# nadongjun/mirbft

Measured on AMD Instinct MI355X. Metric: SHA-256 digests/s (request + batch digests), Actions.Hash stream, higher is better.
Workload: dtype u32

## Files before the change

mirbft_amd/csrc/mirsha_ctx.h:

```cpp
#pragma once
#include <hip/hip_runtime.h>

#include <algorithm>
#include <atomic>
#include <chrono>
#include <condition_variable>
#include <cstdarg>
#include <cstdio>
#include <cstdlib>
#include <cstring>
#include <functional>
#include <mutex>
#include <string>
#include <thread>
#include <vector>

#include "../../include/mirsha.h"
#include "mirsha_host.h"
#include "mirsha_device.h"
#include "mirsha_order.h"
#include "mirsha_sha512.h"
#include "mirsha_sha512_pair.h"
#include "mirsha_sha512_plan.h"

// ... 210 lines not shown
    PinnedBuf stage;
    DevBuf dev, d_out;
    RingOwner ring;
};

struct mirsha_pipeline {
    int device = 0;
    int mode = MIRSHA_PIPELINE_FUSED;
    int hasher = MIRSHA_HASHER_SHA256;
    uint32_t n_req = 0, n_lists = 0, n_entries = 0;
    std::vector<uint32_t> tadj_first, tadj, cbase, expected;
    uint32_t n_tiles = 0, n_groups = 0, n_counters = 0, grid = 0;
    uint32_t pace = 1, list_blocks = 0, tile_waves = 0;
    uint32_t list_tiles = 0;
    uint32_t q_first[mirsha::kFusedMaxQueues + 1] = {};
    uint32_t q_end[mirsha::kFusedMaxQueues] = {};
    uint32_t q_waves[mirsha::kFusedMaxQueues] = {};
    uint32_t tile_blocks = 0;
    uint64_t epoch = 0;
    DevBuf d_tadj_first, d_tadj, d_cbase, d_expected, d_counters, d_ctl, d_trace;
    unsigned long long* h_err = nullptr;
    unsigned long long* d_err = nullptr;
    unsigned long long watchdog = mirsha::kFusedWatchdogTicks;
    uint32_t n_split = 0, split_first = 0, seg_per_tile = 0, seg_nominal_nb = 0;
    std::vector<uint32_t> seg_nb;
    DevBuf d_seg_nb, d_seg_state, d_seg_flags;
    uint64_t seg_runs = 0;
    int fallback = 0;
    uint32_t test_placement = 0;
    DevBuf d_probe;
    bool trace = false;
    std::vector<uint32_t> cidx, cfirst;
    uint32_t uniform = 0;
    std::vector<uint32_t> order;
    DevBuf d_cidx, d_cfirst, d_order;
};

namespace mirsha_api {

int fail(mirsha_ctx* c, int code, const char* fmt, ...);

#define HIP_TRY(c, expr)                                                                    \
    do {                                                                                    \
        hipError_t _e = (expr);                                                             \
        if (_e != hipSuccess)                                                               \
            return fail((c), _e == hipErrorOutOfMemory ? MIRSHA_ENOMEM : MIRSHA_EHIP,       \
                        "%s: %s (%s:%d)", #expr, hipGetErrorString(_e), __FILE__, __LINE__); \
    } while (0)

hipEvent_t take_event(KernelTimer& t);

template <class F>
int timed_launch(mirsha_ctx* c, int which, F&& launch) {
    hipEvent_t e0 = nullptr, e1 = nullptr;
    const bool timed = c->timing && ((c->time_mask >> which) & 1u);
    if (timed) {
        e0 = take_event(c->timers[which]);
        e1 = take_event(c->timers[which]);
        if (e0 && e1) mirsha::next_launch_events() = {e0, e1};
    }
    hipError_t e = launch();
    const bool bound = e0 && e1 && !mirsha::next_launch_events().start;
    mirsha::next_launch_events() = {};
    if (timed && (!bound || e != hipSuccess)) {
        if (e0) c->timers[which].pool.push_back(e0);
        if (e1) c->timers[which].pool.push_back(e1);
    }
    if (e != hipSuccess) return fail(c, MIRSHA_EHIP, "kernel launch: %s", hipGetErrorString(e));
    if (bound) c->timers[which].pending.emplace_back(e0, e1);
    return MIRSHA_OK;
}

inline hipError_t hasher_launch_msgs(const mirsha_ctx* c, const uint8_t* arena, uint64_t arena_len,
                                     const uint64_t* off, const uint32_t* len, const uint32_t* order, uint32_t n,
                                     uint8_t* out, hipStream_t s) {
    if (c->hasher == MIRSHA_HASHER_SHA512_256)
        return mirsha::launch_sha512_msgs(arena, arena_len, off, len, order, n, out, c->variant, s,
                                          &c->sha512_pair_launches);
    return mirsha::launch_msgs(arena, arena_len, off, len, order, n, out, c->variant, s);
}
inline hipError_t hasher_launch_lists(const mirsha_ctx* c, const uint8_t* digests, uint32_t n_digests,
                                      const uint32_t* idx, uint32_t n_entries, const uint32_t* first, uint32_t n_lists,
                                      uint32_t* scratch, uint8_t* out, hipStream_t s) {
    if (c->hasher == MIRSHA_HASHER_SHA512_256)
        return mirsha::launch_sha512_lists(digests, n_digests, idx, n_entries, first, n_lists, scratch, out, s,
                                           &c->sha512_pair_launches);
    return mirsha::launch_lists(digests, n_digests, idx, n_entries, first, n_lists, scratch, out, s);
}

inline const char* hasher_name(int hasher) { return hasher == MIRSHA_HASHER_SHA512_256 ? "sha512_256" : "sha256"; }

inline int sha256_only(mirsha_ctx* c, const char* call) {
    if (!c || c->hasher == MIRSHA_HASHER_SHA256) return MIRSHA_OK;
    return fail(c, MIRSHA_EINVAL, "%s: hasher %s is not built for this call", call, hasher_name(c->hasher));
}

inline int chains_hasher_match(mirsha_ctx* c, const mirsha_chains* ch, const char* call) {
    if (!c || !ch || c->hasher == ch->hasher) return MIRSHA_OK;
    return fail(c, MIRSHA_EINVAL, "%s: the chains hash with %s, the context with %s", call, hasher_name(ch->hasher),
                hasher_name(c->hasher));
}

inline int plan_hasher_match(mirsha_ctx* c, const mirsha_pipeline* p, const char* call) {
    if (!c || !p || c->hasher == p->hasher) return MIRSHA_OK;
    return fail(c, MIRSHA_EINVAL, "%s: the plan hashes with %s, the context with %s", call, hasher_name(p->hasher),
                hasher_name(c->hasher));
}

inline int streams_hasher_match(mirsha_ctx* c, const mirsha_streams* st, const char* call) {
    if (!c || !st || c->hasher == st->hasher) return MIRSHA_OK;
    return fail(c, MIRSHA_EINVAL, "%s: the streams hash with %s, the context with %s", call, hasher_name(st->hasher),
                hasher_name(c->hasher));
// ... 230 lines not shown
```

mirbft_amd/csrc/mirsha_kernels.h:

```cpp
#pragma once
#include <hip/hip_runtime.h>
#include <stdint.h>

namespace mirsha {

constexpr uint32_t kWavesPerBlock = 4;
constexpr uint32_t kBlockThreads = 64 * kWavesPerBlock;
constexpr uint32_t kNullIndex = 0xFFFFFFFFu;

enum : int {
    kVariantLds = 0,
    kVariantDirect = 1,
    kVariantLowOcc = 4,
    kVariantLdsOnly = 5,
    kVariantPair = 6,
    kVariantCu = 10,
};
const char* ab_getenv(const char* name);
inline bool variant_valid(int v) {
    return v == kVariantLds || v == kVariantDirect || v == kVariantLowOcc || v == kVariantLdsOnly || v == kVariantPair ||
           v == kVariantCu;
}
constexpr uint32_t kCuMaxWavesPerSimd = 4;
uint32_t cu_count();
constexpr uint32_t kLowOccTiles = 1024;
constexpr uint32_t kPairMaxGroups = 512;
uint32_t pair_max_groups();

constexpr uint64_t kMaxBufferArena = 0xFFFFFF00ull;
constexpr uint32_t kMaxBufferMsgs = 1u << 27;
hipError_t launch_offsets_scan(void* tmp, size_t& tmp_bytes, const uint32_t* len, uint64_t* off, uint32_t n,
                               hipStream_t s);
struct LaunchEvents {
    hipEvent_t start = nullptr, stop = nullptr;
};
LaunchEvents& next_launch_events();

hipError_t launch_msgs(const uint8_t* arena, uint64_t arena_len, const uint64_t* off,
                       const uint32_t* len, const uint32_t* order, uint32_t n, uint8_t* out,
                       int variant, hipStream_t s);
constexpr uint32_t kMaxListDigests = (1u << 27) - 1u;
constexpr uint32_t kMaxListEntries = (1u << 30) - 1u;
hipError_t launch_lists(const uint8_t* digests, uint32_t n_digests, const uint32_t* idx, uint32_t n_entries,
                        const uint32_t* first, uint32_t n_lists, uint32_t* scratch, uint8_t* out, hipStream_t s);
struct PadBlockKW {
    uint32_t kw[64];
    uint32_t use;
};
PadBlockKW pad_block_kw(uint64_t L);
hipError_t launch_chain(const uint8_t* digests, uint32_t n_digests, const uint32_t* cidx, uint32_t n_entries,
                        const uint32_t* cfirst, uint32_t n_lists, uint8_t* out, hipStream_t s, uint32_t uniform = 0);
hipError_t launch_chain_pair(const uint8_t* digests, uint32_t n_digests, const uint32_t* cidx, uint32_t n_entries,
                             const uint32_t* cfirst, uint32_t n_lists, uint8_t* out, hipStream_t s);
struct OverlapArgs {
    const uint8_t* arena;
    uint64_t arena_len;
    const uint64_t* off;
    const uint32_t* len;
    const uint32_t* order;
    uint32_t n_req;
    uint8_t* req_out;
    const uint8_t* prev_digests;
    uint32_t n_req_prev;
    const uint32_t* cidx;
    uint32_t n_entries;
    const uint32_t* cfirst;
    uint32_t n_lists;
    uint8_t* list_out;
    uint32_t list_waves;
    uint32_t chain_prio;
};
hipError_t launch_msgs_overlap(const OverlapArgs& a, hipStream_t s);
constexpr uint32_t kFusedChunkBlocks = 2;
// ... 63 lines not shown
```

mirbft_amd/csrc/mirsha_kernels.hip:

```cpp
#include <algorithm>
#include <atomic>
#include <cstdlib>
#include <cstdio>
#include <type_traits>

#include "mirsha_device.h"

namespace mirsha {

struct RawChunk {
    uint32_t v[5];
    uint32_t sel;
};

__device__ __forceinline__ void issue_chunk(__amdgpu_buffer_rsrc_t rsrc, uint32_t records, uint32_t o,
                                            uint32_t blk, uint32_t q, bool active, RawChunk& c) {
    const uint32_t addr = o + 64u * blk + 16u * q;
    const uint32_t a = active ? (addr & ~3u) : 0xFFFFFFE0u;
    c.sel = be_sel(addr & 3u);
    if (a + 20u <= records || !active) {
        const auto v = __builtin_amdgcn_raw_buffer_load_b128(rsrc, a, 0, 0);
        c.v[0] = v[0]; c.v[1] = v[1]; c.v[2] = v[2]; c.v[3] = v[3];
        c.v[4] = __builtin_amdgcn_raw_buffer_load_b32(rsrc, a + 16u, 0, 0);
    } else {
        asm volatile(
            "s_nop 4\n\t"
            "buffer_load_dword %0, %5, %6, 0 offen\n\t"
            "buffer_load_dword %1, %5, %6, 0 offen offset:4\n\t"
            "buffer_load_dword %2, %5, %6, 0 offen offset:8\n\t"
            "buffer_load_dword %3, %5, %6, 0 offen offset:12\n\t"
            "buffer_load_dword %4, %5, %6, 0 offen offset:16\n\t"
            "s_waitcnt vmcnt(0)"
            : "=&v"(c.v[0]), "=&v"(c.v[1]), "=&v"(c.v[2]), "=&v"(c.v[3]), "=&v"(c.v[4])
            : "v"(a), "s"(rsrc)
// ... 11 lines not shown
    for (int k = 0; k < 5; k++) c.v[k] = 0u;
    if (active) {
        const uint32_t* p = reinterpret_cast<const uint32_t*>(arena + a);
        if (a + 20u <= records) {
            const u32x4a4 v = *reinterpret_cast<const u32x4a4*>(p);
            c.v[0] = v[0]; c.v[1] = v[1]; c.v[2] = v[2]; c.v[3] = v[3];
            c.v[4] = p[4];
        } else {
#pragma unroll
            for (int k = 0; k < 5; k++)
                if (a + 4u * k + 4u <= records) c.v[k] = p[k];
        }
    }
}

__device__ __forceinline__ void pad_words(uint32_t p, uint32_t L, bool last_block, uint32_t q, uint32_t out[4]) {
    if (p + 16u > L) {
#pragma unroll
        for (int k = 0; k < 4; k++) {
            const int32_t t = (int32_t)(L - (p + 4u * k));
            const uint32_t sh = (uint32_t)t << 3;
            const uint32_t keep = ~(0xFFFFFFFFu >> sh);
            const uint32_t mark = 0x80000000u >> sh;
            const uint32_t part = (out[k] & keep) | mark;
            out[k] = t >= 4 ? out[k] : (t < 0 ? 0u : part);
        }
        if (last_block && q == 3u) {
            out[2] = L >> 29;
            out[3] = L << 3;
        }
    }
}

template <int kWords = 16>
__device__ __forceinline__ void pad_block_uniform(uint32_t w[16], uint32_t soff, uint32_t L, bool last) {
#pragma unroll
    for (int k = 0; k < kWords; k++) {
        const int32_t t = (int32_t)(L - (soff + 4u * k));
        const uint32_t sh = (uint32_t)t << 3;
        uint32_t keep = t >= 4 ? 0xFFFFFFFFu : (t <= 0 ? 0u : ~(0xFFFFFFFFu >> sh));
        uint32_t mark = (t >= 0 && t < 4) ? 0x80000000u >> sh : 0u;
        if (k >= 14 && last) {
            keep = 0u;
            mark = k == 14 ? L >> 29 : L << 3;
        }
        keep = __builtin_amdgcn_readfirstlane(keep);
        mark = __builtin_amdgcn_readfirstlane(mark);
        w[k] = (w[k] & keep) | mark;
    }
}

__device__ __forceinline__ void finish_chunk(const RawChunk& c, uint32_t p, uint32_t L, bool last_block,
                                             uint32_t q, uint32_t out[4]) {
#pragma unroll
    for (int k = 0; k < 4; k++) out[k] = be_word(c.v[k + 1], c.v[k], c.sel);
    pad_words(p, L, last_block, q, out);
}

__device__ __forceinline__ uint32_t lds_slot(uint32_t m, uint32_t q) {
    return m * 4u + (q ^ ((m >> 2) & 3u));
}

__device__ __forceinline__ void store_digest_buf(__amdgpu_buffer_rsrc_t ors, uint32_t msg, const uint32_t st[8]) {
    __builtin_amdgcn_raw_buffer_store_b128(
        (uint32_t __attribute__((ext_vector_type(4)))){__builtin_bswap32(st[0]), __builtin_bswap32(st[1]),
                                                        __builtin_bswap32(st[2]), __builtin_bswap32(st[3])},
        ors, 32u * msg, 0, 0);
    __builtin_amdgcn_raw_buffer_store_b128(
        (uint32_t __attribute__((ext_vector_type(4)))){__builtin_bswap32(st[4]), __builtin_bswap32(st[5]),
                                                        __builtin_bswap32(st[6]), __builtin_bswap32(st[7])},
// ... 90 lines not shown
    asm volatile("s_mov_b32 %0, %1" : "=s"(wnb) : "s"(wave_nb));
    return wnb - blk == 1u;
}

template <bool kFused, bool kBuf>
__device__ __forceinline__ void tile_store(uint8_t* out, uint32_t n, uint32_t msg, const uint32_t st[8]) {
    if constexpr (kFused || kBuf) {
        const __amdgpu_buffer_rsrc_t ors =
            __builtin_amdgcn_make_buffer_rsrc((void*)out, (short)0, (int)(32u * n), 0x00020000);
        if constexpr (kFused)
            store_digest_sc1(ors, msg, st);
        else
            store_digest_buf(ors, msg, st);
    } else {
        store_digest(out, msg, st);
    }
}

template <bool kFused>
__device__ __forceinline__ void block_prio(uint32_t fprio, uint32_t blk) {
    if constexpr (kFused) {
        if (fprio == kPrioBalance)
            balance_prio(blk);
        else if (fprio == kPrioProgress)
            progress_prio(blk);
        else
            fixed_prio(fprio);
    } else {
        progress_prio(blk);
    }
}

constexpr uint32_t kTilePaused = 0, kTileDone = 1;
template <bool kLds, bool kWide, bool kFused = false, bool kDma = false>
__device__ __forceinline__ uint32_t hash_tile(const uint8_t* __restrict__ arena, uint64_t arena_len,
                                          const uint64_t* __restrict__ off, const uint32_t* __restrict__ len,
                                          const uint32_t* __restrict__ order, uint32_t n, uint8_t* __restrict__ out,
                                          uint4* my, uint32_t t, uint32_t lane, uint32_t fprio = 0,
                                          uint32_t b0 = 0u, uint32_t b1 = 0xFFFFFFFFu, uint32_t* st_io = nullptr,
                                          uint32_t lone_sel = 0u, uint4* my2 = nullptr,
                                          unsigned long long* lone_tr = nullptr) {
    __builtin_amdgcn_s_setprio(3);
    const uint32_t slot = t * 64u + lane;
    const bool valid = slot < n;
    const uint32_t slot_c = valid ? slot : n - 1u;
    const uint32_t msg = order ? order[slot_c] : slot_c;
    const uint32_t L_ = len[msg];
    const uint64_t o_ = off[msg];
    const uint32_t L = valid ? L_ : 0u;
    const uint64_t o = valid ? o_ : 0u;
    const uint32_t nb = valid ? blocks_for_len(L) : 0u;
    const uint32_t max_l = wave_max(valid ? L : 0u);
    const uint32_t wave_nb = blocks_for_len(max_l);

    const uint64_t records = (arena_len + 3u) & ~3ull;
    const __amdgpu_buffer_rsrc_t rsrc =
        __builtin_amdgcn_make_buffer_rsrc((void*)arena, (short)0, (int)(uint32_t)records, 0x00020000);
    auto issue = [&](uint64_t mo, uint32_t blk, uint32_t q, bool active, RawChunk& rc) {
        if constexpr (kWide)
            issue_chunk_wide(arena, records, mo, blk, q, active, rc);
        else
            issue_chunk(rsrc, (uint32_t)records, (uint32_t)mo, blk, q, active, rc);
    };

    uint32_t st[8];
#pragma unroll
    for (int i = 0; i < 8; i++) st[i] = (st_io && b0) ? st_io[i] : kH0[i];
    const bool finished = b1 >= wave_nb;

    if constexpr (kLds && !kWide) {
        const uint32_t q = lane & 3u;
        const uint64_t reach = valid ? o + 64ull * wave_nb + 20u : 0ull;
        const bool far = __builtin_amdgcn_ballot_w64(reach > records) == 0;
        const bool aligned = __builtin_amdgcn_ballot_w64(valid && (o & 3u) != 0u) == 0;
        const uint32_t min_l = wave_min(valid ? L : 0xFFFFFFFFu);
        const bool uni = max_l == min_l;
        const int32_t u_last = (int32_t)(min_l - 64u * (wave_nb - 1u));
        const bool tail_ok = uni && u_last <= 16;
        const TailWords tw = tail_words(u_last, min_l);
        uint32_t vo[4], sel[4];
#pragma unroll
        for (int j = 0; j < 4; j++) {
            const uint32_t a = (uint32_t)__shfl((int)(uint32_t)o, 16 * j + (int)(lane >> 2), 64) + 16u * q;
            vo[j] = a & ~3u;
            sel[j] = be_sel(a & 3u);
        }
        auto stage = [&](uint32_t blk, uint32_t w[16], uint32_t ln, bool trim) {
            const uint32_t soff = 64u * blk;
            const uint32_t qq = ln & 3u;
            const bool skip = trim && soff + 16u * qq >= min_l;
            RawChunk rc[4];
            if (far && !trim) {
#pragma unroll
                for (int j = 0; j < 4; j++) {
                    const auto v = __builtin_amdgcn_raw_buffer_load_b128(rsrc, vo[j], soff, 0);
                    rc[j].v[0] = v[0]; rc[j].v[1] = v[1]; rc[j].v[2] = v[2]; rc[j].v[3] = v[3];
                    rc[j].v[4] = 0u;
                }
                if (!aligned) {
#pragma unroll
                    for (int j = 0; j < 4; j++)
                        rc[j].v[4] = __builtin_amdgcn_raw_buffer_load_b32(rsrc, vo[j], soff + 16u, 0);
                }
            } else if (far) {
#pragma unroll
                for (int j = 0; j < 4; j++) {
                    const uint32_t a = skip ? 0xFFFFFFE0u : vo[j] + soff;
                    const auto v = __builtin_amdgcn_raw_buffer_load_b128(rsrc, a, 0, 0);
                    rc[j].v[0] = v[0]; rc[j].v[1] = v[1]; rc[j].v[2] = v[2]; rc[j].v[3] = v[3];
                    rc[j].v[4] = aligned ? 0u : __builtin_amdgcn_raw_buffer_load_b32(rsrc, a + 16u, 0, 0);
                }
// ... 134 lines not shown
            uint32_t w[16];
#pragma unroll
            for (int k = 0; k < 4; k++) {
                const uint4 x = my[lds_slot(lane, (uint32_t)k)];
                w[4 * k + 0] = x.x; w[4 * k + 1] = x.y; w[4 * k + 2] = x.z; w[4 * k + 3] = x.w;
            }
            wave_lds_handoff();
            progress_prio(blk);
            if (blk < nb) compress_asm(st, w);
        }
    } else {
        for (uint32_t blk = 0; blk < wave_nb; blk++) {
            const bool active = blk < nb;
            RawChunk rc[4];
#pragma unroll
            for (int q = 0; q < 4; q++) issue(o, blk, (uint32_t)q, active, rc[q]);
            uint32_t w[16];
#pragma unroll
            for (int q = 0; q < 4; q++)
                finish_chunk(rc[q], 64u * blk + 16u * q, L, blk + 1u == nb, (uint32_t)q, &w[4 * q]);
            progress_prio(blk);
            if (active) compress_asm(st, w);
        }
    }
    if (!finished) {
#pragma unroll
        for (int i = 0; i < 8; i++) st_io[i] = st[i];
        return kTilePaused;
    }
    if (valid) tile_store<kFused, kLds && !kWide>(out, n, msg, st);
    return kTileDone;
}

constexpr uint32_t kMsgWaves = 1;
constexpr uint32_t kMsgOcc = 8, kTileSlots = 256;
template <bool kLds, bool kWide = false>
__global__ __launch_bounds__(64 * kMsgWaves, kWide ? 6 : kMsgOcc) void sha256_msgs_kernel(
    const uint8_t* __restrict__ arena, uint64_t arena_len, const uint64_t* __restrict__ off,
    const uint32_t* __restrict__ len, const uint32_t* __restrict__ order, uint32_t n,
    uint8_t* __restrict__ out) {
    __shared__ uint4 tile[kMsgWaves][kTileSlots];
    const uint32_t lane = threadIdx.x & 63u;
    const uint32_t wv = threadIdx.x >> 6;
    const uint32_t t = blockIdx.x * kMsgWaves + wv;
    if (t * 64u >= n) return;
    hash_tile<kLds, kWide>(arena, arena_len, off, len, order, n, out, tile[wv], t, lane);
}

constexpr uint32_t kCuLds = 96u * 1024u;
__global__ __launch_bounds__(1024, 1) void sha256_msgs_cu_kernel(const uint8_t* __restrict__ arena,
                                                                 uint64_t arena_len,
                                                                 const uint64_t* __restrict__ off,
                                                                 const uint32_t* __restrict__ len,
                                                                 const uint32_t* __restrict__ order, uint32_t n,
                                                                 uint8_t* __restrict__ out) {
    extern __shared__ uint4 cu_lds[];
    const uint32_t lane = threadIdx.x & 63u;
    const uint32_t wv = threadIdx.x >> 6;
    const uint32_t t = blockIdx.x * (blockDim.x >> 6) + wv;
    if (t * 64u >= n) return;
    hash_tile<true, false, false, true>(arena, arena_len, off, len, order, n, out, cu_lds + 256u * wv, t, lane);
}

__device__ __forceinline__ void overlap_chain(const uint8_t* __restrict__ digests, uint32_t n_digests,
                                              const uint32_t* __restrict__ cidx, uint32_t n_entries,
                                              const uint32_t* __restrict__ cfirst, uint32_t n_lists,
                                              uint8_t* __restrict__ list_out, uint32_t g, uint32_t lane,
                                              uint32_t prio_mode) {
    __builtin_amdgcn_s_setprio(3);
    const uint32_t k = g * 64u + lane;
    const bool valid = k < n_lists;
    const uint32_t kc = valid ? k : n_lists - 1u;
    const uint32_t e0_ = cfirst[kc], e1_ = cfirst[kc + 1];
    const uint32_t e0 = valid ? e0_ : 0u;
    const uint32_t c = valid ? e1_ - e0_ : 0u;
    const uint32_t L = 32u * c;
    const uint32_t nb = valid ? blocks_for_len(L) : 0u;
    const uint32_t wave_nb = blocks_for_len(32u * wave_max(c));
    const __amdgpu_buffer_rsrc_t drs = buffer_rsrc(digests, 32u * n_digests);
// ... 886 lines not shown
        const char* m = ab_getenv("MIRSHA_PAIR_MAX_GROUPS");
        return m ? (uint32_t)strtoul(m, nullptr, 10) : kPairMaxGroups;
    }();
    return v;
}

uint32_t cu_count() {
    static std::atomic<uint32_t> cached[64] = {};
    int dev = 0;
    if (hipGetDevice(&dev) != hipSuccess || dev < 0 || dev >= 64) return 256u;
    uint32_t v = cached[dev].load(std::memory_order_relaxed);
    if (!v) {
        int a = 0;
        if (hipDeviceGetAttribute(&a, hipDeviceAttributeMultiprocessorCount, dev) != hipSuccess || a <= 0) a = 256;
        v = (uint32_t)a;
        cached[dev].store(v, std::memory_order_relaxed);
    }
    return v;
}

enum DynLdsKernel { kDynLdsCu, kDynLdsFused, kDynLdsProbe, kDynLdsKernels };
hipError_t dyn_lds_attr(const void* fn, DynLdsKernel form, uint32_t bytes) {
    static std::atomic<uint8_t> done[64][kDynLdsKernels] = {};
    int dev = 0;
    if (hipError_t e = hipGetDevice(&dev)) return e;
    if (dev >= 0 && dev < 64 && done[dev][form].load(std::memory_order_acquire)) return hipSuccess;
    if (hipError_t e = hipFuncSetAttribute(fn, hipFuncAttributeMaxDynamicSharedMemorySize, (int)bytes)) return e;
    if (dev >= 0 && dev < 64) done[dev][form].store(1, std::memory_order_release);
    return hipSuccess;
}

hipError_t launch_msgs(const uint8_t* arena, uint64_t arena_len, const uint64_t* off,
                       const uint32_t* len, const uint32_t* order, uint32_t n, uint8_t* out,
                       int variant, hipStream_t s) {
    if (n == 0) return hipSuccess;
    const uint32_t tiles = (n + 63u) / 64u;
    const uint32_t grid = (tiles + kWavesPerBlock - 1u) / kWavesPerBlock;
    const uint32_t mgrid = (tiles + kMsgWaves - 1u) / kMsgWaves;
    if (arena_len > kMaxBufferArena || n >= kMaxBufferMsgs) {
        launch_k(sha256_msgs_kernel<true, true>, mgrid, 64 * kMsgWaves, 0, s, arena, arena_len, off, len, order, n, out);
        return hipGetLastError();
    }
    if (variant == kVariantPair || (variant == kVariantLds && tiles <= pair_max_groups())) {
        launch_k(sha256_msgs_pair_kernel, tiles, kPairThreads, 0, s, arena, arena_len, off, len, order, n, out);
        return hipGetLastError();
    }
    if (variant == kVariantLowOcc || (variant == kVariantLds && tiles <= kLowOccTiles)) {
        launch_k(sha256_msgs_lowocc_kernel, grid, kBlockThreads, 0, s, arena, arena_len, off, len, order, n, out);
        return hipGetLastError();
    }
    if (variant == kVariantCu || (variant == kVariantLds && tiles <= kCuMaxWavesPerSimd * 4u * cu_count())) {
        const uint32_t k = (tiles + 4u * cu_count() - 1u) / (4u * cu_count());
        const uint32_t wg_waves = 4u * std::min(k, kCuMaxWavesPerSimd);
        const uint32_t cgrid = (tiles + wg_waves - 1u) / wg_waves;
        if (hipError_t e = dyn_lds_attr((const void*)sha256_msgs_cu_kernel, kDynLdsCu, kCuLds)) return e;
        launch_k(sha256_msgs_cu_kernel, cgrid, 64u * wg_waves, kCuLds, s, arena, arena_len, off, len, order, n, out);
        return hipGetLastError();
    }
    if (variant == kVariantDirect)
        launch_k(sha256_msgs_kernel<false>, mgrid, 64 * kMsgWaves, 0, s, arena, arena_len, off, len, order, n, out);
    else
        launch_k(sha256_msgs_kernel<true>, mgrid, 64 * kMsgWaves, 0, s, arena, arena_len, off, len, order, n, out);
    return hipGetLastError();
}

hipError_t launch_msgs_overlap(const OverlapArgs& a, hipStream_t s) {
    const uint32_t tiles = (a.n_req + 63u) / 64u;
    if (a.list_waves + tiles == 0) return hipSuccess;
    if (a.arena_len > kMaxBufferArena || a.n_req >= kMaxBufferMsgs || (a.list_waves && a.n_lists == 0))
        return hipErrorInvalidValue;
    launch_k(sha256_msgs_overlap_kernel, a.list_waves + tiles, 64, 0, s, a);
    return hipGetLastError();
}

hipError_t launch_lists(const uint8_t* digests, uint32_t n_digests, const uint32_t* idx, uint32_t n_entries,
                        const uint32_t* first, uint32_t n_lists, uint32_t* scratch, uint8_t* out, hipStream_t s) {
    if (n_lists == 0) return hipSuccess;
    const uint32_t grid = (n_lists + kBlockThreads - 1u) / kBlockThreads;
    launch_k(sha256_lists_kernel, grid, kBlockThreads, 0, s, digests, n_digests, idx, n_entries, first, n_lists, scratch,
                                                      out);
    return hipGetLastError();
}

PadBlockKW pad_block_kw(uint64_t L) {
    auto rotr = [](uint32_t x, int n) { return (x >> n) | (x << (32 - n)); };
    uint32_t w[64] = {0x80000000u};
    w[14] = (uint32_t)(L >> 29);
    w[15] = (uint32_t)(L << 3);
    for (int j = 16; j < 64; j++) {
        const uint32_t s0 = rotr(w[j - 15], 7) ^ rotr(w[j - 15], 18) ^ (w[j - 15] >> 3);
        const uint32_t s1 = rotr(w[j - 2], 17) ^ rotr(w[j - 2], 19) ^ (w[j - 2] >> 10);
        w[j] = w[j - 16] + s0 + w[j - 7] + s1;
    }
    PadBlockKW p{};
    for (int j = 0; j < 64; j++) p.kw[j] = kK[j] + w[j];
// ... 103 lines not shown
```

mirbft_amd/csrc/mirsha_plan.hip:

```cpp
#include "mirsha_ctx.h"

namespace mirsha_api {

uint32_t uniform_lists(const std::vector<uint32_t>& cidx, const std::vector<uint32_t>& cfirst) {
    const size_t n_lists = cfirst.size() - 1, n = cidx.size();
    if (n_lists == 0 || n == 0 || cfirst[1] == 0) return 0;
    const uint64_t B = cfirst[1];
    if ((n_lists - 1) * B >= n || n_lists * B < n) return 0;
    for (size_t k = 0; k < n_lists; k++)
        if (cfirst[k] != k * B) return 0;
    for (size_t e = 0; e < n; e++)
        if (cidx[e] != e) return 0;
    if (const char* e = mirsha::ab_getenv("MIRSHA_CHAIN_UNIFORM"))
        if (e[0] == '0') return 0;
    return (uint32_t)B;
}

int pipeline_build(mirsha_ctx* c, mirsha_pipeline* p, uint32_t n_req, const uint32_t* idx, const uint32_t* first,
                   uint32_t n_lists, const uint32_t* len) {
    p->n_req = n_req;
    p->n_lists = n_lists;
    p->cfirst.assign(n_lists + 1, 0);
    p->cidx.clear();
    p->cidx.reserve(first[n_lists]);
    std::vector<uint8_t> listed(n_req, 0);
    for (uint32_t k = 0; k < n_lists; k++) {
        for (uint32_t e = first[k]; e < first[k + 1]; e++) {
            if (idx[e] == MIRSHA_NULL_INDEX) continue;
            p->cidx.push_back(idx[e]);
            listed[idx[e]] = 1;
        }
        p->cfirst[k + 1] = (uint32_t)p->cidx.size();
    }
    p->n_entries = (uint32_t)p->cidx.size();
    p->uniform = uniform_lists(p->cidx, p->cfirst);
    p->order.resize(n_req);
    for (uint32_t r = 0; r < n_req; r++) p->order[r] = r;
    std::stable_sort(p->order.begin(), p->order.end(), [&](uint32_t x, uint32_t y) {
        if (listed[x] != listed[y]) return listed[x] > listed[y];
        return len ? host_blocks(len[x]) > host_blocks(len[y]) : false;
    });
    HIP_TRY(c, p->d_cidx.ensure(sizeof(uint32_t) * std::max<uint32_t>(p->n_entries, 1)));
    HIP_TRY(c, p->d_cfirst.ensure(sizeof(uint32_t) * (n_lists + 1)));
    HIP_TRY(c, p->d_order.ensure(sizeof(uint32_t) * std::max<uint32_t>(n_req, 1)));
    if (p->n_entries)
        HIP_TRY(c, hipMemcpyAsync(p->d_cidx.p, p->cidx.data(), sizeof(uint32_t) * p->n_entries, hipMemcpyHostToDevice, c->stream));
    HIP_TRY(c, hipMemcpyAsync(p->d_cfirst.p, p->cfirst.data(), sizeof(uint32_t) * (n_lists + 1), hipMemcpyHostToDevice, c->stream));
    if (n_req)
        HIP_TRY(c, hipMemcpyAsync(p->d_order.p, p->order.data(), sizeof(uint32_t) * n_req, hipMemcpyHostToDevice, c->stream));
    HIP_TRY(c, hipStreamSynchronize(c->stream));
    return MIRSHA_OK;
}

struct PlanKernels {
    hipError_t (*requests)(const mirsha_ctx* c, const mirsha_pipeline* p, const uint8_t* d_arena, uint64_t arena_len,
                           const uint64_t* d_off, const uint32_t* d_len, uint8_t* d_req_out);
    hipError_t (*lists)(const mirsha_ctx* c, const mirsha_pipeline* p, const uint8_t* d_digests, uint8_t* d_list_out);
    hipError_t (*overlap)(const mirsha_ctx* c, const mirsha_pipeline* p, bool tiles, bool chains,
                          const uint8_t* d_arena, uint64_t arena_len, const uint64_t* d_off, const uint32_t* d_len,
                          uint8_t* d_req_out, const uint8_t* d_prev_req, uint8_t* d_prev_batch_out);
};

const PlanKernels kPlanSha256 = {
    [](const mirsha_ctx* c, const mirsha_pipeline* p, const uint8_t* d_arena, uint64_t arena_len, const uint64_t* d_off,
       const uint32_t* d_len, uint8_t* d_req_out) {
        return mirsha::launch_msgs(d_arena, arena_len, d_off, d_len, p->d_order.as<uint32_t>(), p->n_req, d_req_out,
                                   c->variant, c->stream);
    },
    [](const mirsha_ctx* c, const mirsha_pipeline* p, const uint8_t* d_digests, uint8_t* d_list_out) {
        if ((p->n_lists + 63u) / 64u <= mirsha::pair_max_groups())
            return mirsha::launch_chain_pair(d_digests, p->n_req, p->d_cidx.as<uint32_t>(), p->n_entries,
                                             p->d_cfirst.as<uint32_t>(), p->n_lists, d_list_out, c->stream);
        return mirsha::launch_chain(d_digests, p->n_req, p->d_cidx.as<uint32_t>(), p->n_entries,
                                    p->d_cfirst.as<uint32_t>(), p->n_lists, d_list_out, c->stream, p->uniform);
    },
    [](const mirsha_ctx* c, const mirsha_pipeline* p, bool tiles, bool chains, const uint8_t* d_arena,
       uint64_t arena_len, const uint64_t* d_off, const uint32_t* d_len, uint8_t* d_req_out, const uint8_t* d_prev_req,
       uint8_t* d_prev_batch_out) {
        mirsha::OverlapArgs a{};
        a.arena = d_arena;
        a.arena_len = tiles ? arena_len : 0;
        a.off = d_off;
        a.len = d_len;
        a.order = p->d_order.as<uint32_t>();
        a.n_req = tiles ? p->n_req : 0u;
        a.req_out = d_req_out;
        a.prev_digests = d_prev_req;
        a.n_req_prev = p->n_req;
        a.cidx = p->d_cidx.as<uint32_t>();
        a.n_entries = p->n_entries;
        a.cfirst = p->d_cfirst.as<uint32_t>();
        a.n_lists = p->n_lists;
        a.list_out = d_prev_batch_out;
        a.list_waves = chains ? (p->n_lists + 63u) / 64u : 0u;
        if (const char* e = mirsha::ab_getenv("MIRSHA_OVERLAP_CHAIN_PRIO")) a.chain_prio = (uint32_t)atoi(e) & 3u;
        return mirsha::launch_msgs_overlap(a, c->stream);
    },
};

const PlanKernels kPlanSha512 = {
// ... 545 lines not shown
```

mirbft_amd/csrc/mirsha_staging.hip:

```cpp
#include "mirsha_ctx.h"

namespace mirsha_api {





void pmemcpy(void* dst, const void* src, uint64_t n) {
    const int t = n < (1u << 19) ? 1 : (int)std::min<uint64_t>(mirsha::host::threads_for(1ull << 40, 1u << 20), n >> 18);
    mirsha::host::pack_range(static_cast<const uint8_t*>(src), nullptr, nullptr, nullptr, 0, nullptr, 0, n,
                             static_cast<uint8_t*>(dst), t);
}

void fill(const ArenaSrc& src, uint64_t a, uint64_t b, uint8_t* dst) {
    mirsha::host::pack_range(src.base, src.ptr, src.slen, src.sfirst, src.n, src.poff, a, b, dst,
                             mirsha::host::threads_for(b - a, 1u << 20), true);
}

int h2d_arena(mirsha_ctx* c, const ArenaSrc& src, uint8_t* d_arena) {
    if (src.total == 0) return MIRSHA_OK;
    if (src.base && host_pinned(src.base)) {
        HIP_TRY(c, hipMemcpyAsync(d_arena, src.base, src.total, hipMemcpyHostToDevice, c->stream));
        return MIRSHA_OK;
    }
// ... 36 lines not shown
        if (m > a) mirsha::host::pack_range(src - a, nullptr, nullptr, nullptr, 0, nullptr, a, m, dst_at(a),
                                            mirsha::host::threads_for(m - a, 1u << 20));
        if (b > m) mirsha::host::pack_range(src - a, nullptr, nullptr, nullptr, 0, nullptr, m, b, dst_at(m),
                                            mirsha::host::threads_for(b - m, 1u << 20));
    }
    return MIRSHA_OK;
}

struct DrainOnError {
    mirsha_ctx* c;
    bool on = true;
    ~DrainOnError() {
        if (!on) return;
        (void)hipStreamSynchronize(c->stream);
        if (c->xin) (void)hipStreamSynchronize(c->xin);
        if (c->xout) (void)hipStreamSynchronize(c->xout);
    }
};

struct MetaLayout {
    uint64_t off, len, order, idx, first, arena, end;
    MetaLayout(uint32_t n, bool ordered, uint32_t entries, uint32_t n_lists, uint64_t inline_arena) {
        auto al = [](uint64_t x) { return (x + 15u) & ~15ull; };
        off = 0;
        len = al(off + 8ull * n);
        order = al(len + 4ull * n);
        idx = al(order + (ordered ? 4ull * n : 0));
        first = al(idx + 4ull * entries);
        arena = al(first + (n_lists ? 4ull * (n_lists + 1) : 0));
        end = al(arena + inline_arena + (inline_arena ? kArenaSlack : 0));
    }
};

bool meta_fill(const uint64_t* off, const uint32_t* len, uint32_t n, uint64_t shift, uint8_t* h, const MetaLayout& L) {
    std::atomic<uint32_t> lo_b{UINT32_MAX}, hi_b{0};
    uint64_t* ho = reinterpret_cast<uint64_t*>(h + L.off);
    uint32_t* hl = reinterpret_cast<uint32_t*>(h + L.len);
    mirsha::host::parallel_for(n, mirsha::host::threads_for(12ull * n, n), [&](uint32_t a, uint32_t b) {
        uint32_t lo = UINT32_MAX, hi = 0;
        for (uint32_t i = a; i < b; i++) {
            ho[i] = off[i] - shift;
            hl[i] = len[i];
            const uint32_t k = host_blocks(len[i]);
            lo = std::min(lo, k);
            hi = std::max(hi, k);
        }
        uint32_t cur = lo_b.load();
        while (lo < cur && !lo_b.compare_exchange_weak(cur, lo)) {}
        cur = hi_b.load();
        while (hi > cur && !hi_b.compare_exchange_weak(cur, hi)) {}
    });
    return n && lo_b.load() != hi_b.load();
}

hipError_t take_events(mirsha_ctx* c, size_t k) {
    while (c->xev.size() < k) {
        hipEvent_t e = nullptr;
        hipError_t r = hipEventCreateWithFlags(&e, hipEventDisableTiming);
        if (r != hipSuccess) return r;
        c->xev.push_back(e);
    }
    return hipSuccess;
}

constexpr uint64_t kVerdictBits = 8;
inline uint64_t verdict_bytes(uint32_t count) { return kVerdictBits + 8ull * (((uint64_t)count + 63u) / 64u); }

int verify_upload(mirsha_ctx* c, const VerifyArgs& v, uint32_t count) {
    const uint64_t bytes = 32ull * count;
    HIP_TRY(c, c->d_expect.ensure(std::max<uint64_t>(bytes, 32)));
    HIP_TRY(c, c->d_verdict.ensure(verdict_bytes(count)));
    HIP_TRY(c, c->h_verdict.ensure(verdict_bytes(count)));
    const uint8_t* from = v.expected;
    if (!host_pinned(from)) {
        HIP_TRY(c, c->h_expect.ensure(std::max<uint64_t>(bytes, 32)));
        pmemcpy(c->h_expect.p, v.expected, bytes);
        from = c->h_expect.as<uint8_t>();
    }
    HIP_TRY(c, hipMemcpyAsync(c->d_expect.p, from, bytes, hipMemcpyHostToDevice, c->stream));
    return MIRSHA_OK;
}

int verify_queue(mirsha_ctx* c, const uint8_t* d_digests, uint32_t count) {
    uint8_t* dv = c->d_verdict.as<uint8_t>();
// ... 259 lines not shown
    mirsha::host::parallel_for(n, mirsha::host::threads_for(4ull * n, n), [&](uint32_t a, uint32_t b) {
        uint32_t m = 0;
        for (uint32_t i = a; i < b; i++) m = std::max(m, len[i]);
        uint32_t cur = hi.load();
        while (m > cur && !hi.compare_exchange_weak(cur, m)) {}
    });
    return host_blocks(hi.load());
}

constexpr uint32_t kPipeMaxBlocks = 256;

int run_staged(mirsha_ctx* c, const ArenaSrc& src, const uint64_t* off, const uint32_t* len, uint32_t n,
               uint64_t shift, ArenaLayout layout, const uint32_t* idx, const uint32_t* first, uint32_t n_lists,
               uint8_t* req_out, uint8_t* list_out, const VerifyArgs* verify) {
    if (n && layout != kAnyOrder && src.total > kStageChunk && !getenv_flag("MIRSHA_NO_PIPELINED_CALLS") &&
        max_blocks(len, n) <= kPipeMaxBlocks)
        return run_pipelined(c, src, off, len, n, shift, layout == kGapless && !getenv_flag("MIRSHA_NO_OFFSET_SCAN"),
                             idx, first, n_lists, req_out, list_out, verify);
    const uint32_t n_verify = n_lists ? n_lists : n;
    auto t0 = Clock::now();
    c->prof[MIRSHA_PROF_CHUNKS] = 0;
    const uint32_t entries = n_lists ? first[n_lists] : 0u;
    const bool inl = src.total <= kInlineArena;
    HIP_TRY(c, c->d_arena.ensure(inl ? 1 : src.total + kArenaSlack));
    DrainOnError drain{c};
    if (!inl)
        if (int rc = h2d_arena(c, src, c->d_arena.as<uint8_t>())) return rc;
    c->prof[MIRSHA_PROF_PACK] = ms_since(t0);
    t0 = Clock::now();
    const MetaLayout L(n, true, entries, n_lists, inl ? src.total : 0);
    HIP_TRY(c, c->h_meta.ensure(L.end));
    HIP_TRY(c, c->d_meta.ensure(L.end));
    uint8_t* h = c->h_meta.as<uint8_t>();
    const bool ordered = meta_fill(off, len, n, shift, h, L);
    if (ordered) bucket_order(len, n, reinterpret_cast<uint32_t*>(h + L.order));
    if (entries) pmemcpy(h + L.idx, idx, 4ull * entries);
    if (n_lists) pmemcpy(h + L.first, first, 4ull * (n_lists + 1));
    if (inl && src.total) fill(src, 0, src.total, h + L.arena);
    c->prof[MIRSHA_PROF_PLAN] = ms_since(t0);
    t0 = Clock::now();
    HIP_TRY(c, hipMemcpyAsync(c->d_meta.p, h, L.end, hipMemcpyHostToDevice, c->stream));
    if (verify)
        if (int rc = verify_upload(c, *verify, n_verify)) return rc;
    uint8_t* dm = c->d_meta.as<uint8_t>();
    const uint8_t* d_arena = inl ? dm + L.arena : c->d_arena.as<uint8_t>();
    const uint64_t out_bytes = 32ull * ((uint64_t)n + n_lists);
    HIP_TRY(c, c->d_out.ensure(std::max<uint64_t>(out_bytes, 32)));
    uint8_t* d_req = c->d_out.as<uint8_t>();
    uint8_t* d_lst = d_req + 32ull * n;
    if (n) {
        if (int rc = timed_launch(c, 0, [&] {
                return hasher_launch_msgs(c, d_arena, src.total, reinterpret_cast<const uint64_t*>(dm + L.off),
                                          reinterpret_cast<const uint32_t*>(dm + L.len),
                                          ordered ? reinterpret_cast<const uint32_t*>(dm + L.order) : nullptr, n,
                                          d_req, c->stream);
            }))
            return rc;
    }
    if (n_lists) {
        const uint8_t* d_dig = n ? d_req : d_arena;
        const uint32_t n_dig = n ? n : (uint32_t)(src.total / 32u);
        HIP_TRY(c, c->d_scratch.ensure(sizeof(uint32_t) * std::max<uint32_t>(entries, 1)));
        if (int rc = timed_launch(c, 1, [&] {
                return hasher_launch_lists(c, d_dig, n_dig, reinterpret_cast<const uint32_t*>(dm + L.idx), entries,
                                           reinterpret_cast<const uint32_t*>(dm + L.first), n_lists,
                                           c->d_scratch.as<uint32_t>(), d_lst, c->stream);
            }))
            return rc;
    }
    if (verify) {
        if (int rc = verify_queue(c, n_lists ? d_lst : d_req, n_verify)) return rc;
        HIP_TRY(c, hipStreamSynchronize(c->stream));
        c->prof[MIRSHA_PROF_DEVICE] = ms_since(t0);
        t0 = Clock::now();
        verify_publish(c, *verify, n_verify);
    } else if (out_bytes <= kPinnedOutMax) {
        HIP_TRY(c, c->h_outs.ensure(std::max<uint64_t>(out_bytes, 32)));
        HIP_TRY(c, hipMemcpyAsync(c->h_outs.p, d_req, out_bytes, hipMemcpyDeviceToHost, c->stream));
        HIP_TRY(c, hipStreamSynchronize(c->stream));
        c->prof[MIRSHA_PROF_DEVICE] = ms_since(t0);
        t0 = Clock::now();
        if (n) memcpy(req_out, c->h_outs.p, 32ull * n);
        if (n_lists) memcpy(list_out, c->h_outs.as<uint8_t>() + 32ull * n, 32ull * n_lists);
    } else {
        HIP_TRY(c, hipStreamSynchronize(c->stream));
        for (bool& b : c->ring_busy) b = false;
        c->prof[MIRSHA_PROF_DEVICE] = ms_since(t0);
        t0 = Clock::now();
// ... 332 lines not shown
```

Baseline: 5.113 billion.

## Add host-computed uniform-length hint with specialized SHA-256 message tile path

The host detects when all messages share one length and a fixed stride, precomputes padding masks and tail schedule constants, and passes them in a by-value kernel argument struct. A new hinted tile path checks on device that the wave really is uniform and in bounds, then loads through buffer resources with scalar offsets and reads the tail constants straight from the kernarg segment. It also adds per-block priority stepping. If the check fails it falls back to the generic tile, which then has its own tail shortcut disabled. This is meant to remove per-wave length reductions, per-lane padding arithmetic and tail-word computation, at the cost of an extra host-side min/max scan and a larger kernel argument block.

```diff
diff --git a/mirbft_amd/csrc/mirsha_ctx.h b/mirbft_amd/csrc/mirsha_ctx.h
--- a/mirbft_amd/csrc/mirsha_ctx.h
+++ b/mirbft_amd/csrc/mirsha_ctx.h
@@ -266,6 +266,7 @@
     bool trace = false;
     std::vector<uint32_t> cidx, cfirst;
     uint32_t uniform = 0;
+    mirsha::UniformHint hint{};
     std::vector<uint32_t> order;
     DevBuf d_cidx, d_cfirst, d_order;
 };
@@ -307,11 +308,11 @@
 
 inline hipError_t hasher_launch_msgs(const mirsha_ctx* c, const uint8_t* arena, uint64_t arena_len,
                                      const uint64_t* off, const uint32_t* len, const uint32_t* order, uint32_t n,
-                                     uint8_t* out, hipStream_t s) {
+                                     uint8_t* out, hipStream_t s, const mirsha::UniformHint* hint = nullptr) {
     if (c->hasher == MIRSHA_HASHER_SHA512_256)
         return mirsha::launch_sha512_msgs(arena, arena_len, off, len, order, n, out, c->variant, s,
                                           &c->sha512_pair_launches);
-    return mirsha::launch_msgs(arena, arena_len, off, len, order, n, out, c->variant, s);
+    return mirsha::launch_msgs(arena, arena_len, off, len, order, n, out, c->variant, s, hint);
 }
 inline hipError_t hasher_launch_lists(const mirsha_ctx* c, const uint8_t* digests, uint32_t n_digests,
                                       const uint32_t* idx, uint32_t n_entries, const uint32_t* first, uint32_t n_lists,
diff --git a/mirbft_amd/csrc/mirsha_hints.h b/mirbft_amd/csrc/mirsha_hints.h
--- /dev/null
+++ b/mirbft_amd/csrc/mirsha_hints.h
@@ -0,0 +1,66 @@
+#pragma once
+#include <stdint.h>
+
+namespace mirsha {
+
+struct HintTail {
+    uint32_t kw4, kw14, kw15, c4, c14, c15, cs16, cs17, cs19, cs29, cs30;
+};
+
+struct UniformHint {
+    uint32_t valid;
+    uint32_t len;
+    uint32_t stride;
+    uint32_t nb;
+    uint32_t loop_nb;
+    uint32_t tail;
+    uint32_t tail_bytes;
+    uint32_t tail_pad;
+    uint32_t reach;
+    uint32_t keep[4], mark[4];
+    HintTail tw;
+};
+
+namespace hint_detail {
+constexpr uint32_t kK4 = 0x3956c25bu, kK14 = 0x9bdc06a7u, kK15 = 0xc19bf174u;
+inline uint32_t rotr(uint32_t x, int n) { return (x >> n) | (x << (32 - n)); }
+inline uint32_t ssig0(uint32_t x) { return rotr(x, 7) ^ rotr(x, 18) ^ (x >> 3); }
+inline uint32_t ssig1(uint32_t x) { return rotr(x, 17) ^ rotr(x, 19) ^ (x >> 10); }
+}
+
+inline UniformHint make_uniform_hint(uint32_t L, uint64_t stride) {
+    using namespace hint_detail;
+    UniformHint h{};
+    if ((stride & 3u) != 0 || stride > 0xFFFFFFFFull) return h;
+    h.valid = 1;
+    h.len = L;
+    h.stride = (uint32_t)stride;
+    h.nb = (L + 72u) >> 6;
+    const int32_t u = (int32_t)(L - 64u * (h.nb - 1u));
+    h.tail = u <= 16 ? 1u : 0u;
+    h.tail_bytes = (h.tail && u > 0) ? 1u : 0u;
+    h.tail_pad = (h.tail && u < 16) ? 1u : 0u;
+    h.loop_nb = h.tail ? h.nb - 1u : h.nb;
+    h.reach = 64u * h.loop_nb + (h.tail_bytes ? 16u : 0u);
+    for (int k = 0; k < 4; k++) {
+        const int32_t t = u - 4 * k;
+        const uint32_t sh = (uint32_t)(t & 3) << 3;
+        h.keep[k] = t >= 4 ? 0xFFFFFFFFu : (t <= 0 ? 0u : ~(0xFFFFFFFFu >> sh));
+        h.mark[k] = (t >= 0 && t < 4) ? 0x80000000u >> sh : 0u;
+    }
+    HintTail& w = h.tw;
+    w.c4 = u == 16 ? 0x80000000u : 0u;
+    w.c14 = L >> 29;
+    w.c15 = L << 3;
+    w.kw4 = kK4 + w.c4;
+    w.kw14 = kK14 + w.c14;
+    w.kw15 = kK15 + w.c15;
+    w.cs16 = ssig1(w.c14);
+    w.cs17 = ssig1(w.c15);
+    w.cs19 = ssig0(w.c4);
+    w.cs29 = ssig0(w.c14);
+    w.cs30 = ssig0(w.c15) + w.c14;
+    return h;
+}
+
+}
diff --git a/mirbft_amd/csrc/mirsha_kernels.h b/mirbft_amd/csrc/mirsha_kernels.h
--- a/mirbft_amd/csrc/mirsha_kernels.h
+++ b/mirbft_amd/csrc/mirsha_kernels.h
@@ -1,6 +1,8 @@
 #pragma once
 #include <hip/hip_runtime.h>
 #include <stdint.h>
+
+#include "mirsha_hints.h"
 
 namespace mirsha {
 
@@ -38,7 +40,7 @@
 
 hipError_t launch_msgs(const uint8_t* arena, uint64_t arena_len, const uint64_t* off,
                        const uint32_t* len, const uint32_t* order, uint32_t n, uint8_t* out,
-                       int variant, hipStream_t s);
+                       int variant, hipStream_t s, const UniformHint* hint = nullptr);
 constexpr uint32_t kMaxListDigests = (1u << 27) - 1u;
 constexpr uint32_t kMaxListEntries = (1u << 30) - 1u;
 hipError_t launch_lists(const uint8_t* digests, uint32_t n_digests, const uint32_t* idx, uint32_t n_entries,
diff --git a/mirbft_amd/csrc/mirsha_kernels.hip b/mirbft_amd/csrc/mirsha_kernels.hip
--- a/mirbft_amd/csrc/mirsha_kernels.hip
+++ b/mirbft_amd/csrc/mirsha_kernels.hip
@@ -1,5 +1,6 @@
 #include <algorithm>
 #include <atomic>
+#include <cstddef>
 #include <cstdlib>
 #include <cstdio>
 #include <type_traits>
@@ -77,10 +78,10 @@
     }
 }
 
-template <int kWords = 16>
+template <int kWords = 16, int kFirst = 0>
 __device__ __forceinline__ void pad_block_uniform(uint32_t w[16], uint32_t soff, uint32_t L, bool last) {
 #pragma unroll
-    for (int k = 0; k < kWords; k++) {
+    for (int k = kFirst; k < kFirst + kWords; k++) {
         const int32_t t = (int32_t)(L - (soff + 4u * k));
         const uint32_t sh = (uint32_t)t << 3;
         uint32_t keep = t >= 4 ? 0xFFFFFFFFu : (t <= 0 ? 0u : ~(0xFFFFFFFFu >> sh));
@@ -237,7 +238,7 @@
 }
 
 constexpr uint32_t kTilePaused = 0, kTileDone = 1;
-template <bool kLds, bool kWide, bool kFused = false, bool kDma = false>
+template <bool kLds, bool kWide, bool kFused = false, bool kDma = false, bool kTail = true>
 __device__ __forceinline__ uint32_t hash_tile(const uint8_t* __restrict__ arena, uint64_t arena_len,
                                           const uint64_t* __restrict__ off, const uint32_t* __restrict__ len,
                                           const uint32_t* __restrict__ order, uint32_t n, uint8_t* __restrict__ out,
@@ -281,7 +282,7 @@
         const uint32_t min_l = wave_min(valid ? L : 0xFFFFFFFFu);
         const bool uni = max_l == min_l;
         const int32_t u_last = (int32_t)(min_l - 64u * (wave_nb - 1u));
-        const bool tail_ok = uni && u_last <= 16;
+        const bool tail_ok = kTail && uni && u_last <= 16;
         const TailWords tw = tail_words(u_last, min_l);
         uint32_t vo[4], sel[4];
 #pragma unroll
@@ -482,19 +483,134 @@
     return kTileDone;
 }
 
+struct MsgsArgs {
+    const uint8_t* arena;
+    uint64_t arena_len;
+    const uint64_t* off;
+    const uint32_t* len;
+    const uint32_t* order;
+    uint32_t n;
+    uint8_t* out;
+    UniformHint hint;
+};
+__device__ __forceinline__ uint32_t kernarg_u32(uint32_t byte_off) {
+    const auto* p = (const __attribute__((address_space(4))) uint32_t*)__builtin_amdgcn_kernarg_segment_ptr();
+    return p[byte_off / 4u];
+}
+
+__device__ __forceinline__ void progress_prio_uniform(uint32_t blk) {
+    static_assert(kPrioTop == 3, "progress_prio_uniform spells out priorities 3..0");
+    if (blk == 0u) __builtin_amdgcn_s_setprio(3);
+    else if (blk == 1u) __builtin_amdgcn_s_setprio(2);
+    else if (blk == 2u) __builtin_amdgcn_s_setprio(1);
+    else __builtin_amdgcn_s_setprio(0);
+}
+
+__device__ __forceinline__ bool hash_tile_uniform(const uint8_t* __restrict__ arena, uint64_t arena_len,
+                                                  const uint64_t* __restrict__ off, const uint32_t* __restrict__ len,
+                                                  const uint32_t* __restrict__ order, uint32_t n,
+                                                  uint8_t* __restrict__ out, uint4* my, uint32_t t, uint32_t lane,
+                                                  const UniformHint& h) {
+    __builtin_amdgcn_s_setprio(3);
+    t = (uint32_t)__builtin_amdgcn_readfirstlane((int)t);
+    const uint32_t slot = t * 64u + lane;
+    const bool valid = slot < n;
+    const uint32_t slot_c = valid ? slot : n - 1u;
+    const uint32_t msg = order ? order[slot_c] : slot_c;
+    const uint32_t L_ = len[msg];
+    const uint64_t o_ = off[msg];
+    const uint32_t o0 = (uint32_t)__builtin_amdgcn_readfirstlane((int)(uint32_t)o_);
+    const uint32_t o0_hi = (uint32_t)__builtin_amdgcn_readfirstlane((int)(uint32_t)(o_ >> 32));
+    const bool odd = valid & ((L_ != h.len) | (o_ != (((uint64_t)o0_hi << 32 | o0) + (uint64_t)lane * h.stride)));
+    const uint32_t records = (uint32_t)((arena_len + 3u) & ~3ull);
+    const uint32_t last = min(64u, n - t * 64u) - 1u;
+    const uint64_t end = (uint64_t)o0 + (uint64_t)last * h.stride + h.reach;
+    const bool proven = (__builtin_amdgcn_ballot_w64(odd) == 0) & (((o0 | h.stride) & 3u) == 0u) & (o0_hi == 0u) &
+                        ((uint32_t)(end >> 32) == 0u) & ((uint32_t)end <= records);
+    if (!proven) return false;
+
+    const __amdgpu_buffer_rsrc_t rsrc =
+        __builtin_amdgcn_make_buffer_rsrc((void*)arena, (short)0, (int)records, 0x00020000);
+    const uint32_t q = lane & 3u, m = lane >> 2;
+    const uint32_t vbase = o0 + m * h.stride + 16u * q;
+    const uint32_t wslot = lds_slot(m, q);
+    uint32_t st[8];
+#pragma unroll
+    for (int i = 0; i < 8; i++) st[i] = kH0[i];
+    typedef uint32_t u32x4 __attribute__((ext_vector_type(4)));
+    u32x4 tv = {0u, 0u, 0u, 0u};
+    const uint32_t vtail = o0 + lane * h.stride + 64u * h.loop_nb;
+    if (h.tail_bytes && h.loop_nb == 0u) tv = __builtin_amdgcn_raw_buffer_load_b128(rsrc, vtail, 0, 0);
+    for (uint32_t blk = 0; blk < h.loop_nb; blk++) {
+        const uint32_t soff = 64u * blk;
+        u32x4 v[4];
+#pragma unroll
+        for (int j = 0; j < 4; j++)
+            v[j] = __builtin_amdgcn_raw_buffer_load_b128(rsrc, vbase + 16u * (uint32_t)j * h.stride, soff, 0);
+#pragma unroll
+        for (int j = 0; j < 4; j++)
+            my[wslot + 64u * (uint32_t)j] = make_uint4(__builtin_bswap32(v[j][0]), __builtin_bswap32(v[j][1]),
+                                                       __builtin_bswap32(v[j][2]), __builtin_bswap32(v[j][3]));
+        uint32_t w[16];
+        wave_lds_handoff();
+        tile_read_words(my, lane, w);
+        wave_lds_handoff();
+        if (h.tail_bytes && last_block_opaque(h.loop_nb, blk)) tv = __builtin_amdgcn_raw_buffer_load_b128(rsrc, vtail, 0, 0);
+        if (soff + 64u > h.len) {
+            const bool lastb = last_block_opaque(h.nb, blk);
+            pad_block_uniform<4, 0>(w, soff, h.len, lastb);
+            __builtin_amdgcn_sched_barrier(0);
+            pad_block_uniform<4, 4>(w, soff, h.len, lastb);
+            __builtin_amdgcn_sched_barrier(0);
+            pad_block_uniform<4, 8>(w, soff, h.len, lastb);
+            __builtin_amdgcn_sched_barrier(0);
+            pad_block_uniform<4, 12>(w, soff, h.len, lastb);
+        }
+        progress_prio_uniform(blk);
+        compress_asm(st, w);
+    }
+    if (h.tail) {
+        uint32_t w[16];
+        w[0] = __builtin_bswap32(tv[0]); w[1] = __builtin_bswap32(tv[1]);
+        w[2] = __builtin_bswap32(tv[2]); w[3] = __builtin_bswap32(tv[3]);
+        auto arg = [&](size_t field) { return kernarg_u32((uint32_t)(offsetof(MsgsArgs, hint) + field)); };
+        if (h.tail_pad) {
+#pragma unroll
+            for (int k = 0; k < 4; k++)
+                w[k] = (w[k] & arg(offsetof(UniformHint, keep) + 4u * k)) | arg(offsetof(UniformHint, mark) + 4u * k);
+        }
+        constexpr size_t kTw = offsetof(UniformHint, tw);
+        const TailWords tw = {arg(kTw + offsetof(HintTail, kw4)),  arg(kTw + offsetof(HintTail, kw14)),
+                              arg(kTw + offsetof(HintTail, kw15)), arg(kTw + offsetof(HintTail, c4)),
+                              arg(kTw + offsetof(HintTail, c14)),  arg(kTw + offsetof(HintTail, c15)),
+                              arg(kTw + offsetof(HintTail, cs16)), arg(kTw + offsetof(HintTail, cs17)),
+                              arg(kTw + offsetof(HintTail, cs19)), arg(kTw + offsetof(HintTail, cs29)),
+                              arg(kTw + offsetof(HintTail, cs30))};
+        progress_prio_uniform(h.nb - 1u);
+        compress_asm_tail(st, w, tw);
+    }
+    const uint32_t n_end = kernarg_u32((uint32_t)offsetof(MsgsArgs, n));
+    uint8_t* const out_end = reinterpret_cast<uint8_t*>(
+        (uint64_t)kernarg_u32((uint32_t)offsetof(MsgsArgs, out)) |
+        (uint64_t)kernarg_u32((uint32_t)offsetof(MsgsArgs, out) + 4u) << 32);
+    if (slot < n_end) tile_store<false, true>(out_end, n_end, msg, st);
+    return true;
+}
+
 constexpr uint32_t kMsgWaves = 1;
 constexpr uint32_t kMsgOcc = 8, kTileSlots = 256;
-template <bool kLds, bool kWide = false>
-__global__ __launch_bounds__(64 * kMsgWaves, kWide ? 6 : kMsgOcc) void sha256_msgs_kernel(
-    const uint8_t* __restrict__ arena, uint64_t arena_len, const uint64_t* __restrict__ off,
-    const uint32_t* __restrict__ len, const uint32_t* __restrict__ order, uint32_t n,
-    uint8_t* __restrict__ out) {
+template <bool kLds, bool kWide = false, bool kHint = false>
+__global__ __launch_bounds__(64 * kMsgWaves, kWide ? 6 : kMsgOcc) void sha256_msgs_kernel(MsgsArgs a) {
     __shared__ uint4 tile[kMsgWaves][kTileSlots];
     const uint32_t lane = threadIdx.x & 63u;
     const uint32_t wv = threadIdx.x >> 6;
     const uint32_t t = blockIdx.x * kMsgWaves + wv;
-    if (t * 64u >= n) return;
-    hash_tile<kLds, kWide>(arena, arena_len, off, len, order, n, out, tile[wv], t, lane);
+    if (t * 64u >= a.n) return;
+    if constexpr (kHint) {
+        static_assert(kLds && !kWide, "hinted tiles: the narrow LDS loader only");
+        if (hash_tile_uniform(a.arena, a.arena_len, a.off, a.len, a.order, a.n, a.out, tile[wv], t, lane, a.hint)) return;
+    }
+    hash_tile<kLds, kWide, false, false, !kHint>(a.arena, a.arena_len, a.off, a.len, a.order, a.n, a.out, tile[wv], t, lane);
 }
 
 constexpr uint32_t kCuLds = 96u * 1024u;
@@ -1447,13 +1563,14 @@
 
 hipError_t launch_msgs(const uint8_t* arena, uint64_t arena_len, const uint64_t* off,
                        const uint32_t* len, const uint32_t* order, uint32_t n, uint8_t* out,
-                       int variant, hipStream_t s) {
+                       int variant, hipStream_t s, const UniformHint* hint) {
+    const MsgsArgs a{arena, arena_len, off, len, order, n, out, (hint && hint->valid) ? *hint : UniformHint{}};
     if (n == 0) return hipSuccess;
     const uint32_t tiles = (n + 63u) / 64u;
     const uint32_t grid = (tiles + kWavesPerBlock - 1u) / kWavesPerBlock;
     const uint32_t mgrid = (tiles + kMsgWaves - 1u) / kMsgWaves;
     if (arena_len > kMaxBufferArena || n >= kMaxBufferMsgs) {
-        launch_k(sha256_msgs_kernel<true, true>, mgrid, 64 * kMsgWaves, 0, s, arena, arena_len, off, len, order, n, out);
+        launch_k(sha256_msgs_kernel<true, true>, mgrid, 64 * kMsgWaves, 0, s, a);
         return hipGetLastError();
     }
     if (variant == kVariantPair || (variant == kVariantLds && tiles <= pair_max_groups())) {
@@ -1473,9 +1590,11 @@
         return hipGetLastError();
     }
     if (variant == kVariantDirect)
-        launch_k(sha256_msgs_kernel<false>, mgrid, 64 * kMsgWaves, 0, s, arena, arena_len, off, len, order, n, out);
+        launch_k(sha256_msgs_kernel<false>, mgrid, 64 * kMsgWaves, 0, s, a);
+    else if (a.hint.valid)
+        launch_k(sha256_msgs_kernel<true, false, true>, mgrid, 64 * kMsgWaves, 0, s, a);
     else
-        launch_k(sha256_msgs_kernel<true>, mgrid, 64 * kMsgWaves, 0, s, arena, arena_len, off, len, order, n, out);
+        launch_k(sha256_msgs_kernel<true>, mgrid, 64 * kMsgWaves, 0, s, a);
     return hipGetLastError();
 }
 
diff --git a/mirbft_amd/csrc/mirsha_plan.hip b/mirbft_amd/csrc/mirsha_plan.hip
--- a/mirbft_amd/csrc/mirsha_plan.hip
+++ b/mirbft_amd/csrc/mirsha_plan.hip
@@ -34,6 +34,9 @@
     }
     p->n_entries = (uint32_t)p->cidx.size();
     p->uniform = uniform_lists(p->cidx, p->cfirst);
+    p->hint = mirsha::UniformHint{};
+    if (len && n_req && std::all_of(len, len + n_req, [&](uint32_t l) { return l == len[0]; }))
+        p->hint = mirsha::make_uniform_hint(len[0], len[0]);
     p->order.resize(n_req);
     for (uint32_t r = 0; r < n_req; r++) p->order[r] = r;
     std::stable_sort(p->order.begin(), p->order.end(), [&](uint32_t x, uint32_t y) {
@@ -65,7 +68,7 @@
     [](const mirsha_ctx* c, const mirsha_pipeline* p, const uint8_t* d_arena, uint64_t arena_len, const uint64_t* d_off,
        const uint32_t* d_len, uint8_t* d_req_out) {
         return mirsha::launch_msgs(d_arena, arena_len, d_off, d_len, p->d_order.as<uint32_t>(), p->n_req, d_req_out,
-                                   c->variant, c->stream);
+                                   c->variant, c->stream, &p->hint);
     },
     [](const mirsha_ctx* c, const mirsha_pipeline* p, const uint8_t* d_digests, uint8_t* d_list_out) {
         if ((p->n_lists + 63u) / 64u <= mirsha::pair_max_groups())
diff --git a/mirbft_amd/csrc/mirsha_staging.hip b/mirbft_amd/csrc/mirsha_staging.hip
--- a/mirbft_amd/csrc/mirsha_staging.hip
+++ b/mirbft_amd/csrc/mirsha_staging.hip
@@ -92,24 +92,38 @@
     }
 };
 
-bool meta_fill(const uint64_t* off, const uint32_t* len, uint32_t n, uint64_t shift, uint8_t* h, const MetaLayout& L) {
-    std::atomic<uint32_t> lo_b{UINT32_MAX}, hi_b{0};
+bool meta_fill(const uint64_t* off, const uint32_t* len, uint32_t n, uint64_t shift, uint8_t* h, const MetaLayout& L,
+               mirsha::UniformHint* hint) {
+    std::atomic<uint32_t> lo_b{UINT32_MAX}, hi_b{0}, lo_l{UINT32_MAX}, hi_l{0};
     uint64_t* ho = reinterpret_cast<uint64_t*>(h + L.off);
     uint32_t* hl = reinterpret_cast<uint32_t*>(h + L.len);
     mirsha::host::parallel_for(n, mirsha::host::threads_for(12ull * n, n), [&](uint32_t a, uint32_t b) {
-        uint32_t lo = UINT32_MAX, hi = 0;
+        uint32_t lo = UINT32_MAX, hi = 0, lol = UINT32_MAX, hil = 0;
         for (uint32_t i = a; i < b; i++) {
             ho[i] = off[i] - shift;
             hl[i] = len[i];
             const uint32_t k = host_blocks(len[i]);
             lo = std::min(lo, k);
             hi = std::max(hi, k);
-        }
-        uint32_t cur = lo_b.load();
-        while (lo < cur && !lo_b.compare_exchange_weak(cur, lo)) {}
-        cur = hi_b.load();
-        while (hi > cur && !hi_b.compare_exchange_weak(cur, hi)) {}
+            lol = std::min(lol, len[i]);
+            hil = std::max(hil, len[i]);
+        }
+        auto lower = [](std::atomic<uint32_t>& a, uint32_t v) {
+            uint32_t cur = a.load();
+            while (v < cur && !a.compare_exchange_weak(cur, v)) {}
+        };
+        auto raise = [](std::atomic<uint32_t>& a, uint32_t v) {
+            uint32_t cur = a.load();
+            while (v > cur && !a.compare_exchange_weak(cur, v)) {}
+        };
+        lower(lo_b, lo);
+        raise(hi_b, hi);
+        lower(lo_l, lol);
+        raise(hi_l, hil);
     });
+    *hint = mirsha::UniformHint{};
+    if (n && lo_l.load() == hi_l.load())
+        *hint = mirsha::make_uniform_hint(len[0], n > 1 ? off[1] - off[0] : (uint64_t)len[0]);
     return n && lo_b.load() != hi_b.load();
 }
 
@@ -435,7 +449,8 @@
     HIP_TRY(c, c->h_meta.ensure(L.end));
     HIP_TRY(c, c->d_meta.ensure(L.end));
     uint8_t* h = c->h_meta.as<uint8_t>();
-    const bool ordered = meta_fill(off, len, n, shift, h, L);
+    mirsha::UniformHint hint;
+    const bool ordered = meta_fill(off, len, n, shift, h, L, &hint);
     if (ordered) bucket_order(len, n, reinterpret_cast<uint32_t*>(h + L.order));
     if (entries) pmemcpy(h + L.idx, idx, 4ull * entries);
     if (n_lists) pmemcpy(h + L.first, first, 4ull * (n_lists + 1));
@@ -456,7 +471,7 @@
                 return hasher_launch_msgs(c, d_arena, src.total, reinterpret_cast<const uint64_t*>(dm + L.off),
                                           reinterpret_cast<const uint32_t*>(dm + L.len),
                                           ordered ? reinterpret_cast<const uint32_t*>(dm + L.order) : nullptr, n,
-                                          d_req, c->stream);
+                                          d_req, c->stream, &hint);
             }))
             return rc;
     }
```

New measurement: 5.183 billion, median of 6. +1.4%, better.
